# microsoft/OmniParser

Hardware: AMD Instinct MI355X
Metric: screenshots/sec end-to-end (detect+caption) @1920x1080 (higher is better)
Workload: dtype f32 (split-f16x3 MFMA)

## Files before the change

omniparser_amd/csrc/gemm_dma.hip:

```cpp
#include "omni_internal.h"
#include "gemm_common.h"
#include <string.h>
#include <type_traits>

OMNI_RANGE_GUARD_TU()

namespace {

typedef __attribute__((address_space(3))) void lds_void;

struct GemmArgs {
  const unsigned char* x; const unsigned char* w; const float* bias; const float* res; unsigned char* y;
  int M, N, K, nk;
  int ldi, in_coff, ldo, out_coff, ldr, res_coff;
  int mtiles, ntiles, xcd_order, xcd_n;
  float oscale;
  int img_tiles; unsigned w_img_stride; const float* img_oscale;
};

constexpr int GEMM_EPI_SCORES = 3;

#if defined(__AMDGCN__)
struct RowBuf {
  __amdgpu_buffer_rsrc_t r;
  __device__ __forceinline__ RowBuf(const void* base, unsigned bytes) : r(__builtin_amdgcn_make_buffer_rsrc((void*)base, 0, (int)bytes, 0x00020000)) {}
  __device__ __forceinline__ void store16(unsigned off, f32x4 v) const { __builtin_amdgcn_raw_buffer_store_b128(__builtin_bit_cast(u32x4, v), r, (int)off, 0, 0); }
  __device__ __forceinline__ f32x4 load16(unsigned off) const { return __builtin_bit_cast(f32x4, __builtin_amdgcn_raw_buffer_load_b128(r, (int)off, 0, 0)); }
};
#else
struct RowBuf {
  unsigned char* base; unsigned bytes;
  RowBuf(const void* b, unsigned n) : base((unsigned char*)b), bytes(n) {}
  void store16(unsigned off, f32x4 v) const { if (off + 16u <= bytes) *reinterpret_cast<f32x4*>(base + off) = v; }
  f32x4 load16(unsigned off) const { return off + 16u <= bytes ? *reinterpret_cast<const f32x4*>(base + off) : f32x4{0.f, 0.f, 0.f, 0.f}; }
};
#endif

template <int BM, int BN, int WM, int WN, int TM, int TN, int LDS_BYTES, int ACT, bool OSPLIT, bool RES>
__device__ __forceinline__ void gemm_epilogue(f32x16 (&acc)[TM][TN], const GemmArgs& a, unsigned char* lds, int m0, int n0, int wave, int lane, float osc) {
  constexpr int NW = WM * WN;
  const int wm = wave / WN, wn = wave % WN;
  const int hsel = lane >> 5;
  static_assert(TN % 2 == 0, "epilogue stages 64 channels (256 bytes per row) of a wave at a time");
  constexpr int EP = 272;
  static_assert(NW * 32 * EP <= LDS_BYTES, "epilogue staging must fit the LDS ring");
  __syncthreads();
  unsigned char* stg = lds + wave * (32 * EP);
  float amax = 0.0f;
  const int rrow = lane >> 4, chunk = lane & 15;
  const int trows = min(a.M - m0, BM), wc0 = n0 + wn * (BN / WN);
  const RowBuf ybuf(a.y + ((long long)m0 * a.ldo + a.out_coff + wc0) * 4, (unsigned)(trows - 1) * (unsigned)(a.ldo * 4) + (BN / WN) * 4);
  const RowBuf rbuf(RES ? reinterpret_cast<const unsigned char*>(a.res) + ((long long)m0 * a.ldr + a.res_coff + wc0) * 4 : a.y,
                    RES ? (unsigned)(trows - 1) * (unsigned)(a.ldr * 4) + (BN / WN) * 4 : 0u);
  const unsigned yoff = (unsigned)(wm * (BM / WM) + rrow) * (unsigned)(a.ldo * 4) + chunk * 16;
  const unsigned roff = (unsigned)(wm * (BM / WM) + rrow) * (unsigned)(a.ldr * 4) + chunk * 16;
  static_assert(!(RES && OSPLIT), "residual + format-B output is not a layer of this model");
#pragma unroll
  for (int jh = 0; jh < TN / 2; ++jh) {
    const int nw0 = n0 + wn * (BN / WN) + jh * 64;
    f32x4 bq[2][4];
#pragma unroll
// ... 102 lines not shown
      kv[u] = *reinterpret_cast<const float*>(rd + 2 * u * EP + 128);
    }
#pragma unroll
    for (int u = 0; u < 16; ++u) sc[i >> 1] = __builtin_amdgcn_mfma_f32_32x32x2f32(qv[u], kv[u], sc[i >> 1], 0, 0, 0);
    OMNI_WAVE_SYNC();
    __builtin_amdgcn_sched_barrier(0);
  }
  float* hand = reinterpret_cast<float*>(lds + HAND) + wn * 2048;
  if (wm == 1) {
#pragma unroll
    for (int r = 0; r < 2; ++r)
#pragma unroll
      for (int e = 0; e < 16; ++e) hand[(r * 16 + e) * 64 + lane] = sc[r][e];
  }
  __syncthreads();
  if (wm == 0) {
    float* out = reinterpret_cast<float*>(a.y) + ((((long long)img * (a.N / 64) + (n0 / 64 + wn)) * a.img_tiles + chunk) * 1024 + (lane & 31));
#pragma unroll
    for (int e = 0; e < 16; ++e)
      out[((e & 3) + 8 * (e >> 2) + 4 * hsel) * 32] = ((sc[0][e] + sc[1][e]) + hand[e * 64 + lane]) + hand[(16 + e) * 64 + lane];
  }
}

template <int BM, int BN, int WM, int WN, int NSTAGE, int ACT, bool OSPLIT, bool RES, int SCHED = 0>
__global__ __launch_bounds__(WM * WN * 64, 2) void gemm_dma_kernel(GemmArgs a) {
#if defined(__HIP_DEVICE_COMPILE__)
  constexpr int NW = WM * WN;
  constexpr int TM = BM / (32 * WM), TN = BN / (32 * WN);
  constexpr int A_DMA = BM / (8 * NW), B_DMA = BN / (8 * NW);
  constexpr int DPS = A_DMA + B_DMA;
  constexpr int STAGE = (BM + BN) * 128;
  constexpr int NP = TM / 2;
  constexpr int NU = 2 * NP;
  constexpr int NM = 6 * TN;
  static_assert(TM % 2 == 0 && TN >= 1 && A_DMA >= 1 && B_DMA >= 1 && NSTAGE >= 2 && NSTAGE <= 4, "tile / wave grid mismatch");
  static_assert(BM * 128 + (TN - 1) * 4096 < 65536 && (TM - 1) * 4096 < 65536, "ds_read immediate offsets");
  __shared__ __attribute__((aligned(16))) unsigned char lds[NSTAGE * STAGE];

  const int tid = threadIdx.x, lane = tid & 63;
  const int wave = __builtin_amdgcn_readfirstlane(tid >> 6);
  const int wm = wave / WN, wn = wave % WN;
  int mt, nt;
  if (!tile_of_block(blockIdx.x, a.mtiles, a.ntiles, a.xcd_order, a.xcd_n, mt, nt)) return;
  const int m0 = __builtin_amdgcn_readfirstlane(mt) * BM, n0 = __builtin_amdgcn_readfirstlane(nt) * BN;
  const int img = a.img_tiles ? __builtin_amdgcn_readfirstlane(mt / a.img_tiles) : 0;
  const float osc = a.img_oscale ? a.img_oscale[img] : a.oscale;

  const int rsub = lane >> 3, slot = lane & 7;
  unsigned voffA[A_DMA], voffB[B_DMA];
  auto pieceA = [&](int i) { return SCHED == 2 ? wave + NW * i : wave * A_DMA + i; };
#pragma unroll
  for (int i = 0; i < A_DMA; ++i) {
    const int rl = pieceA(i) * 8 + rsub;
    const int rr = min(rl, a.M - 1 - m0);
    voffA[i] = (unsigned)rr * (unsigned)(a.ldi * 4) + (unsigned)((slot ^ ((rl >> 1) & 7)) * 16);
  }
#pragma unroll
  for (int i = 0; i < B_DMA; ++i) {
    const int rl = (wave * B_DMA + i) * 8 + rsub;
    const int rr = min(rl, a.N - 1 - n0);
    voffB[i] = (unsigned)rr * (unsigned)(a.K * 4) + (unsigned)((slot ^ ((rl >> 1) & 7)) * 16);
  }
  const __amdgpu_buffer_rsrc_t rsrcA =
      __builtin_amdgcn_make_buffer_rsrc((void*)(a.x + ((long long)m0 * a.ldi + a.in_coff) * 4), 0, 0x7fffffff, 0x00020000);
  const __amdgpu_buffer_rsrc_t rsrcB =
      __builtin_amdgcn_make_buffer_rsrc((void*)(a.w + (long long)img * a.w_img_stride + (long long)n0 * a.K * 4), 0, 0x7fffffff, 0x00020000);
  auto issue_piece = [&](int kt, int stage, int i) {
    const int so = kt * 128;
    if (i < A_DMA)
      __builtin_amdgcn_raw_ptr_buffer_load_lds(rsrcA, (lds_void*)(lds + stage * STAGE + pieceA(i) * 1024), 16, voffA[i], so, 0, 0);
    else
      __builtin_amdgcn_raw_ptr_buffer_load_lds(rsrcB, (lds_void*)(lds + stage * STAGE + BM * 128 + (wave * B_DMA + i - A_DMA) * 1024), 16,
                                               voffB[i - A_DMA], so, 0, 0);
  };
  auto issue = [&](int kt, int stage) {
#pragma unroll
    for (int i = 0; i < DPS; ++i) issue_piece(kt, stage, i);
  };

  const int swz = (lane >> 1) & 7, hsel = lane >> 5;
  int offA[4], offW[4];
#pragma unroll
  for (int gp = 0; gp < 4; ++gp) {
    const int c = ((((gp >> 1) * 4 + (gp & 1) * 2 + hsel) ^ swz)) * 16;
    offA[gp] = (wm * (BM / WM) + (lane & 31)) * 128 + c;
    offW[gp] = BM * 128 + (wn * (BN / WN) + (lane & 31)) * 128 + c;
  }
  struct AF { f16x8 h[2], l[2]; };
  struct WF { f16x8 h[TN], l[TN]; };
  auto loadA = [&](const unsigned char* st, int g, int ip, AF& f) {
#pragma unroll
    for (int t = 0; t < 2; ++t) {
      f.h[t] = *reinterpret_cast<const f16x8*>(st + offA[g * 2 + 0] + (ip * 2 + t) * 4096);
      f.l[t] = *reinterpret_cast<const f16x8*>(st + offA[g * 2 + 1] + (ip * 2 + t) * 4096);
// ... 16 lines not shown
      for (int e = 0; e < 16; ++e) acc[i][j][e] = 0.0f;

  auto mma = [&](const AF& af, const WF& wf, int ip) {
#pragma unroll
    for (int t = 0; t < 2; ++t)
#pragma unroll
      for (int j = 0; j < TN; ++j)
        acc[ip * 2 + t][j] = __builtin_amdgcn_mfma_f32_32x32x16_f16(wf.h[j], af.h[t], acc[ip * 2 + t][j], 0, 0, 0);
#pragma unroll
    for (int t = 0; t < 2; ++t)
#pragma unroll
      for (int j = 0; j < TN; ++j)
        acc[ip * 2 + t][j] = __builtin_amdgcn_mfma_f32_32x32x16_f16(wf.l[j], af.h[t], acc[ip * 2 + t][j], 0, 0, 0);
#pragma unroll
    for (int t = 0; t < 2; ++t)
#pragma unroll
      for (int j = 0; j < TN; ++j)
        acc[ip * 2 + t][j] = __builtin_amdgcn_mfma_f32_32x32x16_f16(wf.h[j], af.l[t], acc[ip * 2 + t][j], 0, 0, 0);
  };

  const int nk = a.nk;
#pragma unroll
  for (int s = 0; s < NSTAGE - 1; ++s)
    if (s < nk) issue(s, s);
  int stage = 0, nstage = NSTAGE - 1;
  constexpr int IU = SCHED == 1 ? (NU + 1) / 2 : NU;
  constexpr int PPU = (DPS + IU - 1) / IU;
  AF af[2];
  WF wf[2];
  auto slice = [&](int kt, auto more_tag) {
    constexpr bool MORE = decltype(more_tag)::value;
    if constexpr (NSTAGE > 2 && MORE) OMNI_WAIT_VMCNT((NSTAGE - 2) * DPS);
    else OMNI_WAIT_VMCNT(0);
    __builtin_amdgcn_s_barrier();
    const unsigned char* st = lds + stage * STAGE;
    loadW(st, 0, wf[0]);
    loadA(st, 0, 0, af[0]);
#pragma unroll
    for (int u = 0; u < NU; ++u) {
      const int g = u / NP, ip = u % NP;
      int nds = 0;
      if (u + 1 < NU) {
        const int g2 = (u + 1) / NP, ip2 = (u + 1) % NP;
        if (g2 != g) { loadW(st, g2, wf[g2 & 1]); nds += 2 * TN; }
        loadA(st, g2, ip2, af[(u + 1) & 1]);
        nds += 4;
      }
      if constexpr (MORE) {
#pragma unroll
        for (int i = u * PPU; i < (u + 1) * PPU && i < DPS; ++i) issue_piece(kt + NSTAGE - 1, nstage, i);
      }
      mma(af[u & 1], wf[g & 1], ip);
      {
        const int npc = (MORE && u < IU) ? PPU : 0;
#pragma unroll
        for (int k = 0; k < NM; ++k) {
          __builtin_amdgcn_sched_group_barrier(0x8, 1, 0);
          if (k < nds) __builtin_amdgcn_sched_group_barrier(0x100, 1, 0);
          else if (k < nds + npc) __builtin_amdgcn_sched_group_barrier(0x20, 1, 0);
        }
      }
      __builtin_amdgcn_sched_barrier(0);
    }
    stage = stage + 1 == NSTAGE ? 0 : stage + 1;
    nstage = nstage + 1 == NSTAGE ? 0 : nstage + 1;
  };
  if constexpr (SCHED == 2) {
    static_assert(BM == 256 && BN == 256 && WM == 2 && WN == 4 && NSTAGE == 2 && TM == 4 && TN == 2 && A_DMA == 4 && B_DMA == 4, "ping-pong: 256x256 tile, 8 waves");
    OMNI_WAIT_VMCNT(0);
    __builtin_amdgcn_s_barrier();
    if (wm == 1) __builtin_amdgcn_s_barrier();
    auto phase_barrier = [&]() {
      __builtin_amdgcn_sched_barrier(0);
      __builtin_amdgcn_s_barrier();
      __builtin_amdgcn_sched_barrier(0);
    };
    {
      AF afp;
      auto slice_pp = [&](int kt, auto more_tag) {
        constexpr bool MORE = decltype(more_tag)::value;
        const unsigned char* st = lds + stage * STAGE;
#pragma unroll
        for (int u = 0; u < 4; ++u) {
          const int g = u & 1, ip = u >> 1;
          if (u < 2) loadW(st, g, wf[g]);
          loadA(st, g, ip, afp);
          if constexpr (MORE) {
            if (u == 0) { issue_piece(kt + 1, nstage, 0); issue_piece(kt + 1, nstage, 2); }
            if (u == 1) { issue_piece(kt + 1, nstage, A_DMA + 0); issue_piece(kt + 1, nstage, A_DMA + 1); }
            if (u == 2) { issue_piece(kt + 1, nstage, A_DMA + 2); issue_piece(kt + 1, nstage, A_DMA + 3); }
            if (u == 3) { issue_piece(kt + 1, nstage, 1); issue_piece(kt + 1, nstage, 3); }
            if (u == 1) OMNI_WAIT_VMCNT(4);
            if (u == 3) OMNI_WAIT_VMCNT(2);
          } else {
            if (u == 1) OMNI_WAIT_VMCNT(0);
          }
          phase_barrier();
          __builtin_amdgcn_s_setprio(1);
          mma(afp, wf[g], ip);
          __builtin_amdgcn_s_setprio(0);
          phase_barrier();
        }
        stage ^= 1;
        nstage ^= 1;
      };
      int ktp = 0;
      for (; ktp + 1 < nk; ++ktp) slice_pp(ktp, std::true_type{});
      for (; ktp < nk; ++ktp) slice_pp(ktp, std::false_type{});
    }
    if (wm == 0) __builtin_amdgcn_s_barrier();
  } else {
  int kt = 0;
  for (; kt + NSTAGE - 1 < nk; ++kt) slice(kt, std::true_type{});
  for (; kt < nk; ++kt) slice(kt, std::false_type{});
  }

  if constexpr (ACT == GEMM_EPI_SCORES)
    gemm_scores_epilogue<BM, BN, WM, WN, TM, TN, NSTAGE * STAGE>(acc, a, lds, img, __builtin_amdgcn_readfirstlane(mt) - img * a.img_tiles, n0, wave, lane, osc);
  else
    gemm_epilogue<BM, BN, WM, WN, TM, TN, NSTAGE * STAGE, ACT, OSPLIT, RES>(acc, a, lds, m0, n0, wave, lane, osc);
#endif
}

__global__ __launch_bounds__(256) void split_convert_kernel(const float* __restrict__ x, unsigned char* __restrict__ y, long long rows,
                                                            int C, int ldi, int in_coff, int ldo, int out_coff) {
  const int gpr = C / 16;
  const long long idx = (long long)blockIdx.x * blockDim.x + threadIdx.x;
  if (idx >= rows * gpr) return;
  const long long r = idx / gpr;
  const int g = (int)(idx - r * gpr);
  const float* src = x + r * ldi + in_coff + g * 16;
  f32x4 v[4];
#pragma unroll
  for (int q = 0; q < 4; ++q) v[q] = *reinterpret_cast<const f32x4*>(src + q * 4);
  uint2 hi[4], lo[4];
#pragma unroll
  for (int q = 0; q < 4; ++q) {
    float t[4] = {v[q][0], v[q][1], v[q][2], v[q][3]};
    omni_split4(t, hi[q], lo[q]);
  }
  unsigned char* dst = y + (r * ldo + out_coff + g * 16) * 4;
  *reinterpret_cast<u32x4*>(dst) = u32x4{hi[0].x, hi[0].y, hi[1].x, hi[1].y};
  *reinterpret_cast<u32x4*>(dst + 16) = u32x4{hi[2].x, hi[2].y, hi[3].x, hi[3].y};
// ... 115 lines not shown
      gh[kg] = __builtin_bit_cast(f16x8, u32x4{hq[0].x, hq[0].y, hq[1].x, hq[1].y});
      gl[kg] = __builtin_bit_cast(f16x8, u32x4{lq[0].x, lq[0].y, lq[1].x, lq[1].y});
    }
#pragma unroll
    for (int kg = 0; kg < 2; ++kg)
#pragma unroll
      for (int j = 0; j < OB; j += 2) {
        const unsigned char* sw = st + W1B + j * 4096;
        const f16x8 wh0 = *reinterpret_cast<const f16x8*>(sw + fo[kg][0]), wl0 = *reinterpret_cast<const f16x8*>(sw + fo[kg][1]);
        const f16x8 wh1 = *reinterpret_cast<const f16x8*>(sw + 4096 + fo[kg][0]), wl1 = *reinterpret_cast<const f16x8*>(sw + 4096 + fo[kg][1]);
        acc2[0][j] = __builtin_amdgcn_mfma_f32_32x32x16_f16(wh0, gh[kg], acc2[0][j], 0, 0, 0);
        acc2[0][j + 1] = __builtin_amdgcn_mfma_f32_32x32x16_f16(wh1, gh[kg], acc2[0][j + 1], 0, 0, 0);
        acc2[0][j] = __builtin_amdgcn_mfma_f32_32x32x16_f16(wl0, gh[kg], acc2[0][j], 0, 0, 0);
        acc2[0][j + 1] = __builtin_amdgcn_mfma_f32_32x32x16_f16(wl1, gh[kg], acc2[0][j + 1], 0, 0, 0);
        acc2[0][j] = __builtin_amdgcn_mfma_f32_32x32x16_f16(wh0, gl[kg], acc2[0][j], 0, 0, 0);
        acc2[0][j + 1] = __builtin_amdgcn_mfma_f32_32x32x16_f16(wh1, gl[kg], acc2[0][j + 1], 0, 0, 0);
      }
  }
  omni_report_range(amax);
  gemm_epilogue<NW * 32, C, NW, 1, 1, OB, 2 * STAGE, OMNI_ACT_NONE, false, true>(acc2, a.ep, lds, m0, 0, wave, lane, a.ep.oscale);
#endif
}

template <int BM, int BN, int WM, int WN, int NSTAGE>
int launch_tile(GemmArgs& a, int rows_per_img, int act, int osplit, bool scores, hipStream_t s) {
  if (rows_per_img % BM != 0) {
    omni_set_error("gemm_dma: per-image weights need whole %d-row tiles per image (rows per image %d)", BM, rows_per_img);
    return OMNI_E_ARG;
  }
  a.img_tiles = rows_per_img / BM;
  a.mtiles = (a.M + BM - 1) / BM;
  a.ntiles = a.N / BN;
  a.xcd_order = (a.mtiles >= 64 && a.ntiles > 1) ? 1 : 0;
  a.xcd_n = a.xcd_order ? choose_xcd_n(a.ntiles, 4ll * a.N * a.K) : 1;
  dim3 grid(tile_grid(a.mtiles, a.ntiles, a.xcd_order, a.xcd_n)), block(WM * WN * 64);
  const bool res = a.res != nullptr;
  constexpr int SCHED1 = (BM == 256 && BN == 256) ? 1 : 0;
  const char* sched_e = getenv("OMNI_GEMM_SCHED");
  const bool lockstep = sched_e && atoi(sched_e) == 1;
#define OMNI_GD(ACT_, OS_, RES_)                                                                                                   \
  do {                                                                                                                             \
    if constexpr (BM == 256 && BN == 256) {                                                                                        \
      if (!lockstep) { hipLaunchKernelGGL((gemm_dma_kernel<BM, BN, WM, WN, NSTAGE, ACT_, OS_, RES_, 2>), grid, block, 0, s, a); break; }  \
    }                                                                                                                              \
    hipLaunchKernelGGL((gemm_dma_kernel<BM, BN, WM, WN, NSTAGE, ACT_, OS_, RES_, SCHED1>), grid, block, 0, s, a);                  \
  } while (0)
  if (scores) {
    if constexpr (BM == 256 && BN == 256) OMNI_GD(GEMM_EPI_SCORES, false, false);
    else { omni_set_error("gemm_dma: the scores epilogue is built for the 256x256 tile"); return OMNI_E_ARG; }
  }
  else if (act == OMNI_ACT_NONE && !osplit && !res) OMNI_GD(OMNI_ACT_NONE, false, false);
  else if (act == OMNI_ACT_NONE && !osplit && res) OMNI_GD(OMNI_ACT_NONE, false, true);
  else if (act == OMNI_ACT_NONE && osplit && !res) OMNI_GD(OMNI_ACT_NONE, true, false);
  else if (act == OMNI_ACT_GELU && osplit && !res) OMNI_GD(OMNI_ACT_GELU, true, false);
  else if (act == OMNI_ACT_GELU && !osplit && !res) OMNI_GD(OMNI_ACT_GELU, false, false);
#undef OMNI_GD
  else {
    omni_set_error("gemm_dma: unsupported epilogue (act %d, split out %d, residual %d)", act, osplit, (int)res);
    return OMNI_E_ARG;
  }
  return OMNI_OK;
}

}

int omni_launch_gemm_dma(const omni_op_t* op, hipStream_t s) {
  GemmArgs a{};
  a.x = (const unsigned char*)op->p[0]; a.w = (const unsigned char*)op->p[1]; a.bias = (const float*)op->p[2];
  a.res = (const float*)op->p[3]; a.y = (unsigned char*)op->p[4];
  const int B = op->i[0], H = op->i[1], W = op->i[2];
  a.K = op->i[3]; a.ldi = op->i[4]; a.in_coff = op->i[5];
  a.N = op->i[12]; a.ldo = op->i[13]; a.out_coff = op->i[14];
  const int act = op->i[15];
  a.ldr = op->i[16]; a.res_coff = op->i[17];
  const int osplit = op->i[21];
  a.oscale = op->f[1] != 0.0f ? op->f[1] : 1.0f;
  OMNI_REQUIRE(op->dtype == OMNI_F32, "gemm_dma: f32 plans only");
  OMNI_REQUIRE(op->i[28] == 0 || op->i[28] == 1, "gemm_dma: unknown epilogue mode %d (i28)", op->i[28]);
  const bool scores = op->i[28] == 1;
  OMNI_REQUIRE(a.x && a.w && (a.y || scores), "gemm_dma: null pointer");
  if (scores) a.y = (unsigned char*)op->p[7];
  OMNI_REQUIRE(op->i[6] == 1 && op->i[7] == 1 && op->i[8] == 1 && op->i[9] == 0 && op->i[10] == H && op->i[11] == W,
               "gemm_dma: pointwise layers only");
  OMNI_REQUIRE(op->f[0] == 0.0f, "gemm_dma: output scale is not supported");
  const long long M = (long long)B * H * W;
  OMNI_REQUIRE(M > 0 && M < (1ll << 31), "gemm_dma: bad M");
  a.M = (int)M;
  OMNI_REQUIRE(a.K >= 32 && a.K % 32 == 0 && a.N % 128 == 0, "gemm_dma: needs K %% 32 == 0 and N %% 128 == 0 (K %d, N %d)", a.K, a.N);
  OMNI_REQUIRE(a.ldi % 16 == 0 && a.in_coff % 16 == 0, "gemm_dma: split input needs 16-channel aligned ld / offset (%d, %d)", a.ldi, a.in_coff);
  OMNI_REQUIRE(a.ldo % 4 == 0 && a.out_coff % 4 == 0 && (!osplit || (a.ldo % 16 == 0 && a.out_coff % 16 == 0)), "gemm_dma: output alignment");
  OMNI_REQUIRE(!a.res || (a.ldr % 4 == 0 && a.res_coff % 4 == 0), "gemm_dma: residual alignment");
  OMNI_REQUIRE((long long)a.ldi * 4 * 256 < (1ll << 31) && (long long)a.K * 4 * 256 < (1ll << 31) && (long long)a.ldo * 4 * 256 < (1ll << 31) &&
               (long long)a.ldr * 4 * 256 < (1ll << 31), "gemm_dma: row stride too large");
  a.nk = a.K / 32;
  const int rows_per_img = op->i[26];
  OMNI_REQUIRE(rows_per_img >= 0 && op->i[27] >= 0, "gemm_dma: bad per-image weight arguments (%d rows, stride %d)", rows_per_img, op->i[27]);
  if (rows_per_img > 0) {
    OMNI_REQUIRE(a.M % rows_per_img == 0, "gemm_dma: %d rows are no whole number of images of %d rows", a.M, rows_per_img);
    OMNI_REQUIRE(op->i[27] % 16 == 0 && (op->i[27] == 0 || op->i[27] >= a.N * a.K * 4), "gemm_dma: per-image weight stride %d (N %d, K %d)", op->i[27], a.N, a.K);
    a.w_img_stride = (unsigned)op->i[27];
    a.img_oscale = (const float*)op->p[6];
  }
  if (scores) {
    OMNI_REQUIRE(a.y, "gemm_dma: the scores epilogue needs its workspace (p7)");
    OMNI_REQUIRE(rows_per_img > 0 && rows_per_img % 256 == 0, "gemm_dma: the scores epilogue needs whole 256-row chunks per image (i26 = %d)", rows_per_img);
    OMNI_REQUIRE(a.N % 256 == 0, "gemm_dma: the scores epilogue needs N %% 256 == 0 (N %d)", a.N);
    OMNI_REQUIRE(act == OMNI_ACT_NONE && !a.res && !osplit, "gemm_dma: the scores epilogue takes no activation, residual or format-B output");
  }
  int tile = (a.N % 256 == 0) ? 0 : 1;
  {
    const long long mt256 = (a.M + 255) / 256;
    if (mt256 * (a.N / (tile == 0 ? 256 : 128)) < 256) tile = (tile == 0 && mt256 * (a.N / 128) >= 256) ? 1 : 2;
  }
  if (const char* e = getenv("OMNI_GEMM_TILE")) {
    if (!strcmp(e, "256x128")) tile = 1;
    else if (!strcmp(e, "128x128")) tile = 2;
    else if (!strcmp(e, "256x256") && a.N % 256 == 0) tile = 0;
  }
  if (scores) tile = 0;
  int rc;
  if (tile == 0) rc = launch_tile<256, 256, 2, 4, 2>(a, rows_per_img, act, osplit, scores, s);
  else if (tile == 1) rc = launch_tile<256, 128, 4, 2, 3>(a, rows_per_img, act, osplit, false, s);
  else rc = launch_tile<128, 128, 2, 2, 2>(a, rows_per_img, act, osplit, false, s);
  if (rc) return rc;
  OMNI_HIP_CHECK(hipGetLastError());
  return OMNI_OK;
}

int omni_launch_split_convert(const omni_op_t* op, hipStream_t s) {
  const long long rows = (long long)op->i[0] * (op->i[1] > 0 ? op->i[1] : 1);
  const int C = op->i[3], ldi = op->i[4], in_coff = op->i[5], ldo = op->i[13], out_coff = op->i[14];
  OMNI_REQUIRE(op->dtype == OMNI_F32 && op->p[0] && op->p[4], "split_convert: f32 plans, non-null pointers");
  OMNI_REQUIRE(rows > 0 && C > 0 && C % 16 == 0 && ldi % 16 == 0 && in_coff % 16 == 0 && ldo % 16 == 0 && out_coff % 16 == 0,
               "split_convert: 16-channel alignment (C %d, ld %d/%d, off %d/%d)", C, ldi, ldo, in_coff, out_coff);
  const long long total = rows * (C / 16);
  hipLaunchKernelGGL(split_convert_kernel, dim3((unsigned)((total + 255) / 256)), dim3(256), 0, s, (const float*)op->p[0],
                     (unsigned char*)op->p[4], rows, C, ldi, in_coff, ldo, out_coff);
  OMNI_HIP_CHECK(hipGetLastError());
  return OMNI_OK;
}

int omni_launch_mlp_fused(const omni_op_t* op, hipStream_t s) {
  MlpArgs a{};
  a.x = (const unsigned char*)op->p[0]; a.w1 = (const unsigned char*)op->p[1]; a.b1 = (const float*)op->p[2];
  a.w2 = (const unsigned char*)op->p[5];
  a.ep.x = nullptr; a.ep.w = nullptr; a.ep.bias = (const float*)op->p[6]; a.ep.res = (const float*)op->p[3]; a.ep.y = (unsigned char*)op->p[4];
// ... 21 lines not shown
```

omniparser_amd/florence.py:

```python
import contextlib
import json
import math
import os
from pathlib import Path
from types import SimpleNamespace
from typing import Dict, List, Optional

import numpy as np
import torch

from . import _lib as L
from .planner import PlanBuilder, View, torch_dtype

PROMPT_IDS = [0, 2264, 473, 5, 2274, 6190, 116, 2]
TEXT_CAPACITIES = (8, 16, 32, 64)


def text_capacity(n_tokens: int) -> int:
    for c in TEXT_CAPACITIES:
        if n_tokens <= c:
            return c
    raise ValueError(f"a prompt of {n_tokens} tokens exceeds the captioner's limit of {TEXT_CAPACITIES[-1]} prompt tokens "
                     "(bos and eos included)")

# ... 921 lines not shown
            wp, bp = W.dwconv(conv_key)
            pb.keep += [wp, bp]
            pb.add_op(L.make_op(L.OP_DWCONV3_LN, dt,
                                p=[x.ptr, wp.data_ptr(), bp.data_ptr(), hout.ptr, y1.ptr,
                                   W.f32(norm_key + ".weight").data_ptr(), W.f32(norm_key + ".bias").data_ptr()],
                                i={0: x.B, 1: x.H, 2: x.W, 3: x.C, 6: 1 if grp["dma"] else 0}, f={0: 1e-5}))
            hout.fmt = "split" if grp["dma"] else "f32"
            return hout

        self.x_in = pb.alloc(B, R, R, V, zero=True)
        x = self.x_in
        vt = "model.vision_tower."
        self.chan_ws = None
        self.fold_stages = []
        self.stage_out = []
        for s in range(4):
            C = w.embed_dim[s]
            grp["dma"] = use_dma and C % 128 == 0
            k, st, pd = w.patch[s]
            Ho = (x.H + 2 * pd - k) // st + 1
            conv_key = f"{vt}convs.{s}.conv"
            if w.prenorm[s]:
                xn = pb.alloc(B, x.H, x.W, x.C)
                layernorm(f"{vt}convs.{s}.norm", x, xn)
                cur = pb.alloc(B, Ho, Ho, C)
                wp, bp = W.packed(conv_key, lambda: (sd[conv_key + ".weight"], sd[conv_key + ".bias"]))
                pb.conv(xn, wp, bp, cur, k, st, pd)
                pb.release(xn, *([] if x is self.x_in else [x]))
            else:
                t0 = pb.alloc(B, Ho, Ho, C)
                if cap.patch_rows and dt == L.F32 and pb.split and V == 4 and k <= 8 and x is self.x_in:
                    wp, bp = W.cached((conv_key, dt, "patch"), lambda: (pb.pack_weight_patch(sd[conv_key + ".weight"], V),
                                                                         pb.upload(sd[conv_key + ".bias"].float())))
                    pb.conv_patch(x, wp, bp, t0, k, st, pd)
                else:
                    wp, bp = W.cached((conv_key, dt, "pad"), lambda: (pb.pack_weight(sd[conv_key + ".weight"], cin_pad=V),
                                                                       pb.upload(sd[conv_key + ".bias"].float())))
                    pb.conv(x, wp, bp, t0, k, st, pd)
                cur = pb.alloc(B, Ho, Ho, C)
                layernorm(f"{vt}convs.{s}.norm", t0, cur)
                pb.release(t0)
            H = Ho
            N = H * H
            A_, B_ = cur, pb.alloc(B, H, H, C)
            hbuf = pb.alloc(B, H, H, C)
            qkv = pb.alloc(B, H, H, 3 * C)
            att = pb.alloc(B, H, H, C)
            mlp_one = grp["dma"] and cap.fuse_mlp and C == 128 and sd[f"{vt}blocks.{s}.0.spatial_block.ffn.fc1.weight"].shape[0] == 512
            ffn = None if mlp_one else pb.alloc(B, H, H, 4 * C)
# ... 195 lines not shown
        if n == self.B:
            return self
        cp = self._row_plans.pop(n, None)
        if cp is None:
            while len(self._row_plans) >= max(1, int(cap.row_graphs)):
                if dev_sync := (cap.device.type == "cuda"):
                    torch.cuda.synchronize(cap.device)
                self._row_plans.pop(next(iter(self._row_plans)))
            cp = _CaptionPlans(cap, n, self.R, self.T - 1, arena=self, stream=stream)
            cap.row_graph_builds = getattr(cap, "row_graph_builds", 0) + 1
        self._row_plans[n] = cp
        return cp


class _Config(SimpleNamespace):
    pass


class Florence2Captioner:
    fuse_dwln = True
    attn_split_out = True
    fold_chan_proj = True
    chan_scores_in_gemm = True
    fuse_mlp = True
    exact_rows = os.environ.get("OMNI_EXACT_ROWS", "1") != "0"
    row_graphs = int(os.environ.get("OMNI_CAPTION_ROW_GRAPHS", "24"))
    patch_rows = os.environ.get("OMNI_PATCH_ROWS", "1") != "0"
    reuse_activations = True

    long_kv_budget_bytes = 2 ** 30

    def __init__(self, model_dir, device=None, precision: Optional[str] = None, resolution: Optional[int] = None):
        device = L.require_device(device, "Florence2Captioner")
        L.lib()
        self.device = device
        precision = precision or os.environ.get("OMNI_PRECISION", "f32")
        self.dtype = L.F32 if precision == "f32" else L.F16
        self.resolution = int(resolution or os.environ.get("OMNI_CAPTION_RES", "768"))
        self.w = FlorenceWeights(model_dir)
        self.config = _Config(name_or_path=str(model_dir) if "florence" in str(model_dir).lower() else f"florence:{model_dir}",
                              model_type="florence2")
        self.use_graph = os.environ.get("OMNI_HIPGRAPH", "1") != "0"
        self.stream = self._lane_stream(0)
        self._wcache = {}
        self._plans = {}
        self.max_new_tokens = 20
# ... 593 lines not shown
```

omniparser_amd/opwork.py:

```python

NAMES = {1: "conv_igemm/conv_split", 2: "avgpool2", 3: "maxpool", 4: "resize_nearest", 5: "letterbox", 6: "detect_decode", 7: "nms",
         8: "dwconv3", 9: "layernorm", 10: "attn_rows (window / MHA)", 11: "chan_attn", 12: "proj_prep", 13: "assemble", 14: "embed_step",
         15: "attn_decode", 16: "greedy_step", 17: "crop_resize", 18: "dwconv3_ln", 19: "split_convert", 20: "hand_off", 21: "overlay",
         22: "png_pack", 23: "png_deflate", 24: "mlp_fused", 26: "greedy_ctrl_step", 28: "visual_match"}

MFMA_KINDS = (1, 24, 10)


def op_work(op, esz=4):
    i = op.i
    k = op.kind
    if k == 1:
        M, N, K = i[0] * i[10] * i[11], i[12], i[6] * i[7] * i[3]
        if i[25]:
            K = i[6] * i[6] * i[4]
            return 2 * M * N * K, esz * (i[0] * i[1] * i[2] * i[4] + N * K + M * N)
        if i[20] == 2 and i[28] == 1:
            return 2 * M * N * K + 2 * M * N * 16, esz * (M * K + N * K + (M // 256) * (N // 64) * 1024)
        nw = M // i[26] if (i[20] == 2 and i[26] > 0) else 1
        return 2 * M * N * K, esz * (i[0] * i[1] * i[2] * i[3] + nw * N * K + M * N * (2 if op.p[3] else 1))
    if k == 24:
        rows, C, hid = i[0] * max(i[1], 1), i[3], i[12]
        return 4 * rows * C * hid, esz * (3 * rows * C + 2 * C * hid)
    if k in (2, 3, 4):
# ... 41 lines not shown
    if k == 24:
        return (i[0] * max(i[1], 1), i[3], i[12])
    if k in (8, 18):
        return (i[0] * i[1] * i[2], i[3], 0)
    if k == 9:
        return (i[0] * max(i[1], 1), i[3], i[6])
    if k == 10:
        return (i[11] * i[9], i[8] * i[15], i[12])
    if k == 11:
        return (i[0] * i[1], i[3], (2 if i[9] == 1 else 1) if i[8] == 1 else 0)
    if k == 15:
        return (i[10], i[9], i[7] if i[7] > 0 else i[8])
    if k == 28:
        return (i[1], i[3], 0 if i[0] == 0 else i[2])
    return (i[0], i[3], 0)


def op_kernel(op):
    if op.kind == 1:
        if op.i[20] == 2 and op.i[28] == 1:
            return "gemm_dma (scores epilogue)"
        if op.i[20] == 2 and op.i[26] > 0:
            return "gemm_dma (per-image weights)"
        return "gemm_dma" if op.i[20] == 2 else ("conv_split" if op.i[20] else "conv_igemm")
    if op.kind == 11 and op.i[8] == 1:
        return "chan_attn (fold)" if op.i[9] == 1 else "chan_attn (scores + fold)"
    if op.kind == 28:
        return ("visual_match (embed)", "visual_match (partial top-k)", "visual_match (merge)")[op.i[0]] if 0 <= op.i[0] <= 2 else "visual_match"
    return NAMES.get(op.kind, str(op.kind))
```

omniparser_amd/planner.py:

```python
import math
import os
from dataclasses import dataclass
from typing import Optional

import torch

from . import _lib as L


def vec_width(dtype: int) -> int:
    return 4 if dtype == L.F32 else 8


def torch_dtype(dtype: int):
    return torch.float32 if dtype == L.F32 else torch.float16


@dataclass
class View:
    t: torch.Tensor
    coff: int
    C: int
    fmt: str = "f32"

# ... 162 lines not shown
        assert K % 16 == 0
        w2d = w2d.double()
        amax = float(w2d.abs().max())
        k = 0 if amax == 0.0 else 12 - math.floor(math.log2(amax))
        k = max(-24, min(24, k))
        ws = (w2d * (2.0 ** k)).float()
        hi = ws.to(torch.float16)
        lo = (ws - hi.float()).to(torch.float16)
        return torch.cat([hi.view(cout, K // 16, 16), lo.view(cout, K // 16, 16)], -1).contiguous(), 2.0 ** -k

    KPERM16 = (0, 1, 2, 3, 8, 9, 10, 11, 4, 5, 6, 7, 12, 13, 14, 15)

    def pack_weight_dma(self, w: torch.Tensor, kperm: bool = False) -> torch.Tensor:
        w2d = w.detach().float().reshape(w.shape[0], -1)
        if kperm:
            cout, K = w2d.shape
            assert K % 16 == 0
            w2d = w2d.view(cout, K // 16, 16)[:, :, list(self.KPERM16)].reshape(cout, K).contiguous()
        t, oscale = self.split_f16_b(w2d)
        t = self.upload(t)
        t.omni_fmt, t.omni_oscale = 2, oscale
        return t

    def pack_weight(self, w: torch.Tensor, cin_pad: Optional[int] = None) -> torch.Tensor:
        w = w.detach().float()
        cout, cin, kh, kw = w.shape
        if cin_pad and cin_pad > cin:
            w = torch.cat([w, w.new_zeros(cout, cin_pad - cin, kh, kw)], 1)
        w = w.permute(0, 2, 3, 1).reshape(cout, -1)
        cin_eff = max(cin, cin_pad or 0)
        if self.split and self.dtype == L.F32 and cin_eff % 32 == 0 and cin_eff * kh * kw >= 128:
            t = self.upload(self.split_f16(w))
            t.omni_fmt = 1
            return t
        return self.upload(w.to(torch_dtype(self.dtype)))

    def conv(self, x: View, w_packed: torch.Tensor, bias: Optional[torch.Tensor], out: View, k: int, s: int = 1,
             p: Optional[int] = None, act: int = L.ACT_NONE, res: Optional[View] = None, scale: float = 0.0,
             out_split: bool = False):
        p = k // 2 if p is None else p
        Ho = (x.H + 2 * p - k) // s + 1
        Wo = (x.W + 2 * p - k) // s + 1
        assert (out.B, out.H, out.W) == (x.B, Ho, Wo), ((out.B, out.H, out.W), (x.B, Ho, Wo))
        cout = out.C
        wfmt = getattr(w_packed, "omni_fmt", 0) if self.dtype == L.F32 else 0
        if wfmt:
            assert w_packed.dtype == torch.float16 and w_packed.numel() == 2 * cout * k * k * x.C and x.C % 32 == 0, \
                (tuple(w_packed.shape), cout, k, x.C)
        else:
            assert tuple(w_packed.shape) == (cout, k * k * x.C), (tuple(w_packed.shape), cout, k, x.C)
        if wfmt == 2:
            assert k == 1 and s == 1 and p == 0 and scale == 0.0 and cout % 128 == 0, "format-B weights: pointwise layers, Cout % 128 == 0"
            assert x.fmt == "split", "the LDS-DMA GEMM reads a pre-split input: its producer must emit format B (or insert split_convert)"
            assert x.ld % 16 == 0 and x.coff % 16 == 0 and not (out_split and (res is not None or out.ld % 16 or out.coff % 16))
        else:
            assert x.fmt == "f32" and not out_split, "register-staged conv kernels read and write f32"
        if res is not None:
            assert (res.B, res.H, res.W, res.C) == (out.B, out.H, out.W, out.C) and res.fmt == "f32"
        b = None
        if bias is not None:
            b = bias if bias.device == self.device and bias.dtype == torch.float32 else self.upload(bias.detach().float())
            ent = _TENSORS.get(b.data_ptr())
            if ent is None or ent[0]() is not b:
                _register(b, "const")
            self.keep.append(b)
            assert b.numel() == cout
        if self.ws is None and (self.device.type == "cuda" or self.workspace_on_host):
            self.ws = self.raw((self.ws_kib * 256,), torch.float32, zero=False)
        if self.cnt is None and self.ws is not None and self.n_cnt and wfmt == 1:
            self.cnt = self.raw((self.n_cnt,), torch.int32, zero=True)
        cnt = self.cnt if (wfmt == 1 and self.cnt is not None) else None
        tune = (0, 0)
        if wfmt == 1 and self.conv_tuning:
            tune = tuple(self.conv_tuning.get(conv_key(x.B * Ho * Wo, cout, k * k * x.C, k, s), (0, 0)))
        op = L.make_op(
            L.OP_CONV, self.dtype,
            p=[x.ptr, w_packed.data_ptr(), b.data_ptr() if b is not None else None,
               res.ptr if res is not None else None, out.ptr, self.ws.data_ptr() if self.ws is not None else None,
               cnt.data_ptr() if cnt is not None else None],
            i={0: x.B, 1: x.H, 2: x.W, 3: x.C, 4: x.ld, 5: x.coff, 6: k, 7: k, 8: s, 9: p, 10: Ho, 11: Wo,
               12: cout, 13: out.ld, 14: out.coff, 15: act,
               16: res.ld if res is not None else 0, 17: res.coff if res is not None else 0,
               19: self.ws_kib if self.ws is not None else 0, 20: wfmt, 21: 1 if out_split else 0,
               22: tune[0], 23: tune[1], 24: cnt.numel() if cnt is not None else 0},
            f={0: scale, 1: getattr(w_packed, "omni_oscale", 0.0) if wfmt == 2 else 0.0})
        self.ops.append(op)
        self.keep.append(w_packed)
        out.fmt = "split" if out_split else "f32"
        M = x.B * Ho * Wo
        esz = 4 if self.dtype == L.F32 else 2
        self.flops += 2 * M * cout * k * k * x.C
        self.bytes += esz * (x.B * x.H * x.W * x.C + w_packed.numel() // (2 if wfmt else 1) + M * cout * (2 if res is not None else 1))
        return out

    @staticmethod
    def weight_rows(w_packed: torch.Tensor, row0: int, rows: int) -> torch.Tensor:
        assert getattr(w_packed, "omni_fmt", 0) == 2 and 0 <= row0 and row0 + rows <= w_packed.shape[0]
        t = w_packed[row0:row0 + rows]
        t.omni_fmt, t.omni_oscale = 2, w_packed.omni_oscale
        return t

    def conv_per_image(self, x: View, w_img: torch.Tensor, scales: torch.Tensor, bias: Optional[torch.Tensor], out: View,
                       res: Optional[View], rows_per_img: int):
        cout, K = out.C, x.C
        M = x.B * x.H * x.W
        assert self.dtype == L.F32 and x.fmt == "split" and x.ld % 16 == 0 and x.coff % 16 == 0 and cout % 128 == 0 and K % 32 == 0
        assert (out.B, out.H, out.W) == (x.B, x.H, x.W) and M % rows_per_img == 0
# ... 151 lines not shown
```

Baseline: 13.26.

## Add implicit-GEMM gather feed to LDS-DMA GEMM for Florence stage convolutions

Extends the LDS-DMA GEMM kernel with a gather mode that computes per-row input offsets and per-tap validity masks, so k>1 strided convolutions can stream their input directly into LDS. Out-of-bounds taps are redirected to an offset the buffer resource range check rejects, so they load zeros. Florence vision stage convs 1-3 now pre-split their normalized input and use format-B packed weights on this path, replacing the register-staged conv kernel. This adds a split_convert pass per stage and restricts the path to bias-only f32 output.

```diff
diff --git a/omniparser_amd/csrc/gemm_dma.hip b/omniparser_amd/csrc/gemm_dma.hip
--- a/omniparser_amd/csrc/gemm_dma.hip
+++ b/omniparser_amd/csrc/gemm_dma.hip
@@ -19,6 +19,15 @@
 };
 
 constexpr int GEMM_EPI_SCORES = 3;
+
+struct ConvGemmArgs : GemmArgs {
+  int Hi, Wi, Ho, Wo, stride, pad, kw, cpt;
+  unsigned xbytes;
+};
+constexpr unsigned GATHER_OOB = 0xffff0000u;
+#if !defined(__AMDGCN__)
+const unsigned char gather_zeros[16] = {};
+#endif
 
 #if defined(__AMDGCN__)
 struct RowBuf {
@@ -36,7 +45,7 @@
 };
 #endif
 
-template <int BM, int BN, int WM, int WN, int TM, int TN, int LDS_BYTES, int ACT, bool OSPLIT, bool RES>
+template <int BM, int BN, int WM, int WN, int TM, int TN, int LDS_BYTES, int ACT, bool OSPLIT, bool RES, bool CONV = false>
 __device__ __forceinline__ void gemm_epilogue(f32x16 (&acc)[TM][TN], const GemmArgs& a, unsigned char* lds, int m0, int n0, int wave, int lane, float osc) {
   constexpr int NW = WM * WN;
   const int wm = wave / WN, wn = wave % WN;
@@ -185,8 +194,8 @@
   }
 }
 
-template <int BM, int BN, int WM, int WN, int NSTAGE, int ACT, bool OSPLIT, bool RES, int SCHED = 0>
-__global__ __launch_bounds__(WM * WN * 64, 2) void gemm_dma_kernel(GemmArgs a) {
+template <int BM, int BN, int WM, int WN, int NSTAGE, int ACT, bool OSPLIT, bool RES, int SCHED = 0, bool CONV = false>
+__global__ __launch_bounds__(WM * WN * 64, 2) void gemm_dma_kernel(std::conditional_t<CONV, ConvGemmArgs, GemmArgs> a) {
 #if defined(__HIP_DEVICE_COMPILE__)
   constexpr int NW = WM * WN;
   constexpr int TM = BM / (32 * WM), TN = BN / (32 * WN);
@@ -212,11 +221,26 @@
   const int rsub = lane >> 3, slot = lane & 7;
   unsigned voffA[A_DMA], voffB[B_DMA];
   auto pieceA = [&](int i) { return SCHED == 2 ? wave + NW * i : wave * A_DMA + i; };
+  unsigned tapsA[CONV ? A_DMA : 1];
 #pragma unroll
   for (int i = 0; i < A_DMA; ++i) {
     const int rl = pieceA(i) * 8 + rsub;
     const int rr = min(rl, a.M - 1 - m0);
-    voffA[i] = (unsigned)rr * (unsigned)(a.ldi * 4) + (unsigned)((slot ^ ((rl >> 1) & 7)) * 16);
+    if constexpr (CONV) {
+      const int r = m0 + rr, b = r / (a.Ho * a.Wo), rem = r - b * (a.Ho * a.Wo), oy = rem / a.Wo, ox = rem - oy * a.Wo;
+      const int iy0 = oy * a.stride - a.pad, ix0 = ox * a.stride - a.pad;
+      voffA[i] = (unsigned)((b * a.Hi + iy0) * a.Wi + ix0) * (unsigned)(a.ldi * 4) + (unsigned)((slot ^ ((rl >> 1) & 7)) * 16);
+      unsigned m = 0;
+      const int ntap = a.K / (a.cpt * 32);
+      for (int t = 0, ky = 0, kx = 0; t < ntap; ++t) {
+        const bool in = iy0 + ky >= 0 && iy0 + ky < a.Hi && ix0 + kx >= 0 && ix0 + kx < a.Wi;
+        m |= in ? 1u << t : 0u;
+        if (++kx == a.kw) { kx = 0; ++ky; }
+      }
+      tapsA[i] = m;
+    } else {
+      voffA[i] = (unsigned)rr * (unsigned)(a.ldi * 4) + (unsigned)((slot ^ ((rl >> 1) & 7)) * 16);
+    }
   }
 #pragma unroll
   for (int i = 0; i < B_DMA; ++i) {
@@ -224,15 +248,39 @@
     const int rr = min(rl, a.N - 1 - n0);
     voffB[i] = (unsigned)rr * (unsigned)(a.K * 4) + (unsigned)((slot ^ ((rl >> 1) & 7)) * 16);
   }
-  const __amdgpu_buffer_rsrc_t rsrcA =
-      __builtin_amdgcn_make_buffer_rsrc((void*)(a.x + ((long long)m0 * a.ldi + a.in_coff) * 4), 0, 0x7fffffff, 0x00020000);
+  __amdgpu_buffer_rsrc_t rsrcA;
+  if constexpr (CONV) rsrcA = __builtin_amdgcn_make_buffer_rsrc((void*)(a.x + (long long)a.in_coff * 4), 0, (int)a.xbytes, 0x00020000);
+  else rsrcA = __builtin_amdgcn_make_buffer_rsrc((void*)(a.x + ((long long)m0 * a.ldi + a.in_coff) * 4), 0, 0x7fffffff, 0x00020000);
+  int g_tap = 0, g_cg = 0, g_kx = 0;
+  unsigned g_delta = 0;
+  auto gather_next = [&]() {
+    if constexpr (CONV) {
+      g_delta += 128;
+      if (++g_cg == a.cpt) {
+        g_cg = 0; ++g_tap;
+        g_delta += (unsigned)(a.ldi * 4) - (unsigned)(a.cpt * 128);
+        if (++g_kx == a.kw) { g_kx = 0; g_delta += (unsigned)((a.Wi - a.kw) * (a.ldi * 4)); }
+      }
+    }
+  };
   const __amdgpu_buffer_rsrc_t rsrcB =
       __builtin_amdgcn_make_buffer_rsrc((void*)(a.w + (long long)img * a.w_img_stride + (long long)n0 * a.K * 4), 0, 0x7fffffff, 0x00020000);
   auto issue_piece = [&](int kt, int stage, int i) {
     const int so = kt * 128;
-    if (i < A_DMA)
-      __builtin_amdgcn_raw_ptr_buffer_load_lds(rsrcA, (lds_void*)(lds + stage * STAGE + pieceA(i) * 1024), 16, voffA[i], so, 0, 0);
-    else
+    if (i < A_DMA) {
+      if constexpr (CONV) {
+        const unsigned off = ((tapsA[i] >> g_tap) & 1u) ? voffA[i] + g_delta : GATHER_OOB;
+#if defined(__AMDGCN__)
+        __builtin_amdgcn_raw_ptr_buffer_load_lds(rsrcA, (lds_void*)(lds + stage * STAGE + pieceA(i) * 1024), 16, off, 0, 0, 0);
+#else
+        const bool in_range = (unsigned long long)off + 16u <= a.xbytes;
+        __builtin_amdgcn_raw_ptr_buffer_load_lds(in_range ? rsrcA : __builtin_amdgcn_make_buffer_rsrc((void*)gather_zeros, 0, 16, 0x00020000),
+                                                 (lds_void*)(lds + stage * STAGE + pieceA(i) * 1024), 16, in_range ? off : 0u, 0, 0, 0);
+#endif
+      } else {
+        __builtin_amdgcn_raw_ptr_buffer_load_lds(rsrcA, (lds_void*)(lds + stage * STAGE + pieceA(i) * 1024), 16, voffA[i], so, 0, 0);
+      }
+    } else
       __builtin_amdgcn_raw_ptr_buffer_load_lds(rsrcB, (lds_void*)(lds + stage * STAGE + BM * 128 + (wave * B_DMA + i - A_DMA) * 1024), 16,
                                                voffB[i - A_DMA], so, 0, 0);
   };
@@ -295,7 +343,7 @@
   const int nk = a.nk;
 #pragma unroll
   for (int s = 0; s < NSTAGE - 1; ++s)
-    if (s < nk) issue(s, s);
+    if (s < nk) { issue(s, s); gather_next(); }
   int stage = 0, nstage = NSTAGE - 1;
   constexpr int IU = SCHED == 1 ? (NU + 1) / 2 : NU;
   constexpr int PPU = (DPS + IU - 1) / IU;
@@ -335,6 +383,7 @@
       }
       __builtin_amdgcn_sched_barrier(0);
     }
+    if constexpr (MORE) gather_next();
     stage = stage + 1 == NSTAGE ? 0 : stage + 1;
     nstage = nstage + 1 == NSTAGE ? 0 : nstage + 1;
   };
@@ -374,6 +423,7 @@
           __builtin_amdgcn_s_setprio(0);
           phase_barrier();
         }
+        if constexpr (MORE) gather_next();
         stage ^= 1;
         nstage ^= 1;
       };
@@ -391,7 +441,7 @@
   if constexpr (ACT == GEMM_EPI_SCORES)
     gemm_scores_epilogue<BM, BN, WM, WN, TM, TN, NSTAGE * STAGE>(acc, a, lds, img, __builtin_amdgcn_readfirstlane(mt) - img * a.img_tiles, n0, wave, lane, osc);
   else
-    gemm_epilogue<BM, BN, WM, WN, TM, TN, NSTAGE * STAGE, ACT, OSPLIT, RES>(acc, a, lds, m0, n0, wave, lane, osc);
+    gemm_epilogue<BM, BN, WM, WN, TM, TN, NSTAGE * STAGE, ACT, OSPLIT, RES, CONV>(acc, a, lds, m0, n0, wave, lane, osc);
 #endif
 }
 
@@ -553,8 +603,9 @@
 #endif
 }
 
-template <int BM, int BN, int WM, int WN, int NSTAGE>
-int launch_tile(GemmArgs& a, int rows_per_img, int act, int osplit, bool scores, hipStream_t s) {
+template <int BM, int BN, int WM, int WN, int NSTAGE, class ARGS>
+int launch_tile(ARGS& a, int rows_per_img, int act, int osplit, bool scores, hipStream_t s) {
+  constexpr bool CONV = std::is_same_v<ARGS, ConvGemmArgs>;
   if (rows_per_img % BM != 0) {
     omni_set_error("gemm_dma: per-image weights need whole %d-row tiles per image (rows per image %d)", BM, rows_per_img);
     return OMNI_E_ARG;
@@ -576,6 +627,17 @@
     }                                                                                                                              \
     hipLaunchKernelGGL((gemm_dma_kernel<BM, BN, WM, WN, NSTAGE, ACT_, OS_, RES_, SCHED1>), grid, block, 0, s, a);                  \
   } while (0)
+  if constexpr (CONV) {
+    if (scores || act != OMNI_ACT_NONE || osplit || res) {
+      omni_set_error("gemm_dma: the gather feed (i29) takes bias and f32 output only (act %d, split out %d, residual %d)", act, osplit, (int)res);
+      return OMNI_E_ARG;
+    }
+    if constexpr (BM == 256 && BN == 256) {
+      if (!lockstep) { hipLaunchKernelGGL((gemm_dma_kernel<BM, BN, WM, WN, NSTAGE, OMNI_ACT_NONE, false, false, 2, true>), grid, block, 0, s, a); return OMNI_OK; }
+    }
+    hipLaunchKernelGGL((gemm_dma_kernel<BM, BN, WM, WN, NSTAGE, OMNI_ACT_NONE, false, false, SCHED1, true>), grid, block, 0, s, a);
+    return OMNI_OK;
+  } else
   if (scores) {
     if constexpr (BM == 256 && BN == 256) OMNI_GD(GEMM_EPI_SCORES, false, false);
     else { omni_set_error("gemm_dma: the scores epilogue is built for the 256x256 tile"); return OMNI_E_ARG; }
@@ -596,7 +658,7 @@
 }
 
 int omni_launch_gemm_dma(const omni_op_t* op, hipStream_t s) {
-  GemmArgs a{};
+  ConvGemmArgs a{};
   a.x = (const unsigned char*)op->p[0]; a.w = (const unsigned char*)op->p[1]; a.bias = (const float*)op->p[2];
   a.res = (const float*)op->p[3]; a.y = (unsigned char*)op->p[4];
   const int B = op->i[0], H = op->i[1], W = op->i[2];
@@ -611,10 +673,28 @@
   const bool scores = op->i[28] == 1;
   OMNI_REQUIRE(a.x && a.w && (a.y || scores), "gemm_dma: null pointer");
   if (scores) a.y = (unsigned char*)op->p[7];
-  OMNI_REQUIRE(op->i[6] == 1 && op->i[7] == 1 && op->i[8] == 1 && op->i[9] == 0 && op->i[10] == H && op->i[11] == W,
-               "gemm_dma: pointwise layers only");
+  OMNI_REQUIRE(op->i[29] == 0 || op->i[29] == 1, "gemm_dma: unknown feed mode %d (i29)", op->i[29]);
+  const bool gather = op->i[29] == 1;
+  OMNI_REQUIRE(gather || (op->i[6] == 1 && op->i[7] == 1 && op->i[8] == 1 && op->i[9] == 0 && op->i[10] == H && op->i[11] == W),
+               "gemm_dma: pointwise layers only (or the gather feed, i29 = 1)");
   OMNI_REQUIRE(op->f[0] == 0.0f, "gemm_dma: output scale is not supported");
-  const long long M = (long long)B * H * W;
+  long long M = (long long)B * H * W;
+  if (gather) {
+    const int KH = op->i[6], KW = op->i[7], st = op->i[8], pd = op->i[9], Ho = op->i[10], Wo = op->i[11], Cin = a.K;
+    OMNI_REQUIRE(B > 0 && H > 0 && W > 0 && KH >= 1 && KW >= 1 && KH * KW <= 25 && st >= 1 && pd >= 0, "gemm_dma: bad convolution geometry (k %dx%d s %d p %d)", KH, KW, st, pd);
+    OMNI_REQUIRE(H + 2 * pd >= KH && W + 2 * pd >= KW && Ho == (H + 2 * pd - KH) / st + 1 && Wo == (W + 2 * pd - KW) / st + 1,
+                 "gemm_dma: output size %dx%d does not follow from input %dx%d, k %dx%d s %d p %d", Ho, Wo, H, W, KH, KW, st, pd);
+    OMNI_REQUIRE(Cin >= 32 && Cin % 32 == 0, "gemm_dma: the gather feed needs Cin %% 32 == 0 (Cin %d)", Cin);
+    OMNI_REQUIRE(M < (1ll << 31) && (long long)KH * KW * Cin < (1ll << 24), "gemm_dma: the gather feed's input or K is too large");
+    const long long xbytes = ((M - 1) * a.ldi + Cin) * 4;
+    OMNI_REQUIRE(xbytes <= (long long)GATHER_OOB, "gemm_dma: the gather feed addresses its input with 32-bit offsets (%lld bytes)", xbytes);
+    OMNI_REQUIRE(op->i[26] == 0 && op->i[28] == 0 && !a.res && act == OMNI_ACT_NONE && !osplit,
+                 "gemm_dma: the gather feed takes one weight matrix, bias and f32 output only");
+    a.Hi = H; a.Wi = W; a.Ho = Ho; a.Wo = Wo; a.stride = st; a.pad = pd; a.kw = KW; a.cpt = Cin / 32;
+    a.xbytes = (unsigned)xbytes;
+    a.K = KH * KW * Cin;
+    M = (long long)B * Ho * Wo;
+  }
   OMNI_REQUIRE(M > 0 && M < (1ll << 31), "gemm_dma: bad M");
   a.M = (int)M;
   OMNI_REQUIRE(a.K >= 32 && a.K % 32 == 0 && a.N % 128 == 0, "gemm_dma: needs K %% 32 == 0 and N %% 128 == 0 (K %d, N %d)", a.K, a.N);
@@ -649,10 +729,20 @@
     else if (!strcmp(e, "256x256") && a.N % 256 == 0) tile = 0;
   }
   if (scores) tile = 0;
+  if (gather && op->i[22]) {
+    OMNI_REQUIRE(op->i[22] >= 1 && op->i[22] <= 3 && (op->i[22] != 1 || a.N % 256 == 0), "gemm_dma: bad tile %d (i22) for N %d", op->i[22], a.N);
+    tile = op->i[22] - 1;
+  }
   int rc;
-  if (tile == 0) rc = launch_tile<256, 256, 2, 4, 2>(a, rows_per_img, act, osplit, scores, s);
-  else if (tile == 1) rc = launch_tile<256, 128, 4, 2, 3>(a, rows_per_img, act, osplit, false, s);
-  else rc = launch_tile<128, 128, 2, 2, 2>(a, rows_per_img, act, osplit, false, s);
+  GemmArgs& g = a;
+  if (gather) {
+    if (tile == 0) rc = launch_tile<256, 256, 2, 4, 2>(a, 0, act, osplit, false, s);
+    else if (tile == 1) rc = launch_tile<256, 128, 4, 2, 3>(a, 0, act, osplit, false, s);
+    else rc = launch_tile<128, 128, 2, 2, 2>(a, 0, act, osplit, false, s);
+  }
+  else if (tile == 0) rc = launch_tile<256, 256, 2, 4, 2>(g, rows_per_img, act, osplit, scores, s);
+  else if (tile == 1) rc = launch_tile<256, 128, 4, 2, 3>(g, rows_per_img, act, osplit, false, s);
+  else rc = launch_tile<128, 128, 2, 2, 2>(g, rows_per_img, act, osplit, false, s);
   if (rc) return rc;
   OMNI_HIP_CHECK(hipGetLastError());
   return OMNI_OK;
diff --git a/omniparser_amd/florence.py b/omniparser_amd/florence.py
--- a/omniparser_amd/florence.py
+++ b/omniparser_amd/florence.py
@@ -967,9 +967,17 @@
             conv_key = f"{vt}convs.{s}.conv"
             if w.prenorm[s]:
                 xn = pb.alloc(B, x.H, x.W, x.C)
+                stages = getattr(cap, "stage_conv_dma_stages", Florence2Captioner.stage_conv_dma_stages)
+                gather = grp["dma"] and bool(cap.stage_conv_dma) and s in stages and pb.runs_kernels and pb.conv_gather_ok(xn, C, k)
                 layernorm(f"{vt}convs.{s}.norm", x, xn)
+                if gather:
+                    pb.split_convert(xn)
                 cur = pb.alloc(B, Ho, Ho, C)
-                wp, bp = W.packed(conv_key, lambda: (sd[conv_key + ".weight"], sd[conv_key + ".bias"]))
+                if gather:
+                    wp, bp = W.cached((conv_key, dt, "gather"), lambda: (pb.pack_weight_conv_dma(sd[conv_key + ".weight"]),
+                                                                          pb.upload(sd[conv_key + ".bias"].float())))
+                else:
+                    wp, bp = W.packed(conv_key, lambda: (sd[conv_key + ".weight"], sd[conv_key + ".bias"]))
                 pb.conv(xn, wp, bp, cur, k, st, pd)
                 pb.release(xn, *([] if x is self.x_in else [x]))
             else:
@@ -1211,6 +1219,8 @@
     attn_split_out = True
     fold_chan_proj = True
     chan_scores_in_gemm = True
+    stage_conv_dma = True
+    stage_conv_dma_stages = (1, 2, 3)
     fuse_mlp = True
     exact_rows = os.environ.get("OMNI_EXACT_ROWS", "1") != "0"
     row_graphs = int(os.environ.get("OMNI_CAPTION_ROW_GRAPHS", "24"))
diff --git a/omniparser_amd/opwork.py b/omniparser_amd/opwork.py
--- a/omniparser_amd/opwork.py
+++ b/omniparser_amd/opwork.py
@@ -87,6 +87,8 @@
             return "gemm_dma (scores epilogue)"
         if op.i[20] == 2 and op.i[26] > 0:
             return "gemm_dma (per-image weights)"
+        if op.i[20] == 2 and op.i[29] == 1:
+            return "gemm_dma (gather feed)"
         return "gemm_dma" if op.i[20] == 2 else ("conv_split" if op.i[20] else "conv_igemm")
     if op.kind == 11 and op.i[8] == 1:
         return "chan_attn (fold)" if op.i[9] == 1 else "chan_attn (scores + fold)"
diff --git a/omniparser_amd/planner.py b/omniparser_amd/planner.py
--- a/omniparser_amd/planner.py
+++ b/omniparser_amd/planner.py
@@ -208,6 +208,24 @@
         t.omni_fmt, t.omni_oscale = 2, oscale
         return t
 
+    @property
+    def runs_kernels(self) -> bool:
+        return self.device.type == "cuda" or self.workspace_on_host
+
+    GATHER_MAX_BYTES = 0xffff0000
+
+    def conv_gather_ok(self, x: View, cout: int, k: int) -> bool:
+        span = ((x.B * x.H * x.W - 1) * x.ld + x.C) * 4
+        return (self.dtype == L.F32 and x.C % 32 == 0 and cout % 128 == 0 and x.ld % 16 == 0 and x.coff % 16 == 0
+                and 1 < k * k <= 25 and span <= self.GATHER_MAX_BYTES)
+
+    def pack_weight_conv_dma(self, w: torch.Tensor) -> torch.Tensor:
+        w = w.detach().float()
+        t, oscale = self.split_f16_b(w.permute(0, 2, 3, 1).reshape(w.shape[0], -1))
+        t = self.upload(t)
+        t.omni_fmt, t.omni_oscale = 2, oscale
+        return t
+
     def pack_weight(self, w: torch.Tensor, cin_pad: Optional[int] = None) -> torch.Tensor:
         w = w.detach().float()
         cout, cin, kh, kw = w.shape
@@ -223,7 +241,7 @@
 
     def conv(self, x: View, w_packed: torch.Tensor, bias: Optional[torch.Tensor], out: View, k: int, s: int = 1,
              p: Optional[int] = None, act: int = L.ACT_NONE, res: Optional[View] = None, scale: float = 0.0,
-             out_split: bool = False):
+             out_split: bool = False, tile: int = 0):
         p = k // 2 if p is None else p
         Ho = (x.H + 2 * p - k) // s + 1
         Wo = (x.W + 2 * p - k) // s + 1
@@ -235,7 +253,11 @@
                 (tuple(w_packed.shape), cout, k, x.C)
         else:
             assert tuple(w_packed.shape) == (cout, k * k * x.C), (tuple(w_packed.shape), cout, k, x.C)
-        if wfmt == 2:
+        gather = wfmt == 2 and k > 1
+        if gather:
+            assert x.fmt == "split" and self.conv_gather_ok(x, cout, k) and scale == 0.0 and act == L.ACT_NONE and res is None and not out_split, \
+                "format-B weights with k > 1: the gather feed (conv_gather_ok), bias and f32 output only"
+        elif wfmt == 2:
             assert k == 1 and s == 1 and p == 0 and scale == 0.0 and cout % 128 == 0, "format-B weights: pointwise layers, Cout % 128 == 0"
             assert x.fmt == "split", "the LDS-DMA GEMM reads a pre-split input: its producer must emit format B (or insert split_convert)"
             assert x.ld % 16 == 0 and x.coff % 16 == 0 and not (out_split and (res is not None or out.ld % 16 or out.coff % 16))
@@ -268,7 +290,7 @@
                12: cout, 13: out.ld, 14: out.coff, 15: act,
                16: res.ld if res is not None else 0, 17: res.coff if res is not None else 0,
                19: self.ws_kib if self.ws is not None else 0, 20: wfmt, 21: 1 if out_split else 0,
-               22: tune[0], 23: tune[1], 24: cnt.numel() if cnt is not None else 0},
+               22: tile if gather else tune[0], 23: tune[1], 24: cnt.numel() if cnt is not None else 0, 29: 1 if gather else 0},
             f={0: scale, 1: getattr(w_packed, "omni_oscale", 0.0) if wfmt == 2 else 0.0})
         self.ops.append(op)
         self.keep.append(w_packed)
```

New measurement: 13.32 (median of 6 runs). Within noise of the previous version (+0.5%).
